# hungdinhxuan/real-time-deepfake-speech-detection

Hardware: AMD Instinct MI355X
Metric: utterances/sec (4 s @ 16 kHz) (higher is better)
Workload: dtype fp16

## Files before the change

### real-time-deepfake-speech-detection_amd/csrc/afx_engine.hip

```cpp
#include <hip/hip_runtime.h>

#include <algorithm>
#include <cmath>
#include <cstdarg>
#include <cstdio>
#include <cstring>
#include <string>
#include <unordered_map>
#include <unordered_set>
#include <vector>

#include "../../include/afx.h"
#include "afx_common.h"
#include "afx_kernels.h"
#include "afx_aasist.h"
#include "afx_entry.h"

using namespace afx;

static thread_local char g_err[512] = "";
int afx::fail(const char* fmt, ...) {
  va_list ap;
  va_start(ap, fmt);
  vsnprintf(g_err, sizeof g_err, fmt, ap);
// ... 29 lines not shown
  for (int i = 0; i < 7; ++i) {
    L = L >= kConvK[i] ? (L - kConvK[i]) / kConvS[i] + 1 : 0;
    T[i] = L;
  }
}

__global__ void bn_fold_kernel(const float* w, const float* b, const float* m, const float* v, float eps, int n,
                               float* scale, float* shift) {
  const int i = blockIdx.x * blockDim.x + threadIdx.x;
  if (i < n) {
    const float s = w[i] / sqrtf(v[i] + eps);
    scale[i] = s;
    shift[i] = b[i] - m[i] * s;
  }
}

__global__ void absmax_kernel(const float* x, int n, float* out) {
  float m = 0.f;
  for (int i = threadIdx.x; i < n; i += blockDim.x) m = fmaxf(m, fabsf(x[i]));
  __shared__ float red[4];
  m = wave_max(m);
  if ((threadIdx.x & 63) == 0) red[threadIdx.x >> 6] = m;
  __syncthreads();
  if (threadIdx.x == 0) out[0] = fmaxf(fmaxf(red[0], red[1]), fmaxf(red[2], red[3]));
}

struct FT {
  float* p = nullptr;
  size_t n = 0;
  std::vector<int64_t> shape;
};

struct TapRec {
  float* p = nullptr;
  size_t cap = 0, n = 0;
};

struct LnW {
  const float *g = nullptr, *b = nullptr;
  float scale = kS3ScaleBounded;
};
struct ConvLayer {
  const float* bias = nullptr;
  LnW ln;
  const float *w0 = nullptr, *gn_g = nullptr, *gn_b = nullptr;
};
struct TrunkLayer {
  void *wqkv = nullptr, *wo = nullptr, *w1 = nullptr, *w2 = nullptr;
  float* bqkv = nullptr;
  LnW ln1, ln2;
  const float *bo = nullptr, *b1 = nullptr, *b2 = nullptr;
};
struct ConfFF {
  void *w1, *w2;
  LnW ln;
  const float *b1, *b2;
};
struct ConfBlock {
  ConfFF ff[2];
  void *wqkv, *wout, *pw1, *pw2;
  float *bn_scale, *bn_shift;
  void* rel_h;
  float* chain_prm[3];
  LnW attn_ln, conv_ln, post_ln;
  const float *bout, *bpw1, *bpw2;
  const float* rel32;
  const float *dw_w, *dw_b;
};

struct Profiler;

struct afx_engine {
  afx_config cfg;
  bool s3 = false;
  Profiler* prof = nullptr;
  int dt;
  size_t hsz;
  std::vector<void*> allocs;
  std::unordered_map<std::string, FT> f;
  std::unordered_set<std::string> loaded;
  bool finalized = false;
  bool taps_on = false;
  int posconv_sliding = 1;
  int conf_attn_mfma = 1;
  int fuse_conformer = 1;
  int fuse_conv_ln = 1;
  int gemm_small_deep = 1;
  int concurrent = 0;
  int last_objective = 0;
  std::unordered_map<std::string, TapRec> taps;
  int* nonfinite = nullptr;

  void* convw[7] = {nullptr};
  void* conv0pack = nullptr;
  void* projw = nullptr;
  void* posw = nullptr;
  float* pos_norm = nullptr;
  ConvLayer conv[7];
  LnW feat_ln, enc_ln;
  const float *proj_b = nullptr, *pos_b = nullptr;
  std::vector<TrunkLayer> layers;
  int E = 0, Ep = 0, heads = 0, dh = 0, inner = 0, FF = 0, FFp = 0, C2 = 0, C2p = 0, ck = 0, nblk = 0;
  void* conf_ll = nullptr;
  float conf_bn_scale = 1.f, conf_bn_shift = 0.f;
  const float *ll_b = nullptr, *class_token = nullptr, *fc5_w = nullptr, *fc5_b = nullptr;
  std::vector<ConfBlock> blk;
  AasistWeights aw;

  void* walloc(size_t rows, size_t k) { return dalloc(rows * k * hsz + (s3 ? rows * 4 : 0)); }
  float* wscale(const void* w, size_t rows, size_t k) const { return s3 ? (float*)((char*)w + rows * k * 4) : nullptr; }
  void* dalloc(size_t bytes) {
    void* p = nullptr;
    if (hipMalloc(&p, bytes ? bytes : 16) != hipSuccess) return nullptr;
    allocs.push_back(p);
    return p;
  }
  const float* F(const std::string& k) const {
    auto it = f.find(k);
    return it == f.end() ? nullptr : it->second.p;
  }
};

static void prof_forget(afx_engine* e);
extern "C" const char* afx_last_error(void) { return g_err; }
extern "C" const char afx_build_id_str[];
extern "C" const char* afx_build_id(void) { return afx_build_id_str; }
extern "C" const char* afx_version(void) {
  static char v[96] = "";
  if (!v[0]) snprintf(v, sizeof v, "afx 0.4 (gfx950) build %s hip %d.%d.%d", afx_build_id_str, HIP_VERSION_MAJOR, HIP_VERSION_MINOR, HIP_VERSION_PATCH);
  return v;
}
extern "C" int afx_hip_versions(int* build, int* runtime) {
  if (build) *build = HIP_VERSION;
  int rt = 0;
  if (hipRuntimeGetVersion(&rt) != hipSuccess) return fail("afx_hip_versions: hipRuntimeGetVersion failed");
  if (runtime) *runtime = rt;
  return 0;
}

extern "C" int afx_create(const afx_config* cfg, afx_handle* out) {
  if (!cfg || !out) return fail("afx_create: null argument");
  const bool head_only = cfg->arch == AFX_ARCH_CONFORMER_HEAD;
  if (!head_only && (cfg->n_layers < 1 || cfg->n_layers > 24))
    return fail("Number of layers must be at least 1 and at most 24.");
  if (cfg->dtype != AFX_DT_BF16 && cfg->dtype != AFX_DT_FP16 && cfg->dtype != AFX_DT_FP32 && cfg->dtype != AFX_DT_FP16X3)
    return fail("afx_create: unknown dtype %d", cfg->dtype);
  if (cfg->arch < AFX_ARCH_SSL || cfg->arch > AFX_ARCH_CONFORMER_HEAD) return fail("afx_create: unknown arch %d", cfg->arch);
  if (cfg->extractor_mode != AFX_EXTRACTOR_LAYER_NORM && cfg->extractor_mode != AFX_EXTRACTOR_GROUP_NORM)
    return fail("afx_create: unknown extractor_mode %d", cfg->extractor_mode);
  if (cfg->extractor_mode == AFX_EXTRACTOR_GROUP_NORM && cfg->pre_emphasis)
    return fail("afx_create: fused pre-emphasis is built for the layer_norm extractor only");
  int ndev = 0;
  if (hipGetDeviceCount(&ndev) != hipSuccess || ndev == 0)
    return fail("afx_create: no HIP device visible -- this library has no CPU fallback");
  afx_engine* e = new afx_engine();
  e->cfg = *cfg;
  e->s3 = cfg->dtype == AFX_DT_FP16X3;
  e->dt = e->s3 ? (int)DT_FP32 : cfg->dtype;
  e->hsz = dtype_size(e->dt);
  const int nl = head_only ? 0 : cfg->n_layers;
  e->cfg.n_layers = nl;
  e->layers.resize(nl);
  bool ok = true;
  ok &= (e->nonfinite = (int*)e->dalloc(16)) != nullptr && hipMemset(e->nonfinite, 0, 16) == hipSuccess;
  if (!head_only) {
    for (int i = 1; i < 7; ++i) ok &= (e->convw[i] = e->walloc(kC, (size_t)kC * kConvK[i])) != nullptr;
// ... 820 lines not shown
  const hipStream_t s = cx.s;
  const int dt = e->dt;
  const int* T = w.T;
  if (T[6] < 1) return fail("afx_forward: %d samples are too few for one output frame (need >= 400)", L);
  const ConvLayer& c0 = e->conv[0];
  const bool gn = e->cfg.extractor_mode == AFX_EXTRACTOR_GROUP_NORM;
  if (!l5)
    KOK(cx.timed(PC_CONV0, 2.0 * B * T[0] * kC * kConvK[0], [&] {
      if (gn)
        return launch_conv0_groupnorm(wave, B, L, T[0], c0.w0, c0.gn_g, c0.gn_b, kLnEps,
                                      w.gn_stats, w.bufA, dt, s);
      if (e->s3) {
        const float sc = cx.s3_ok(w.bufA) ? c0.ln.scale : 0.f;
        cx.s3_set(w.bufA, sc);
        return launch_conv0(wave, B, L, T[0], c0.w0, c0.bias, c0.ln.g, c0.ln.b, e->cfg.pre_emphasis, e->cfg.pre_emphasis_coef, w.bufA, DT_FP16X3, s, e->conv0pack, sc);
      }
      return launch_conv0(wave, B, L, T[0], c0.w0, c0.bias, c0.ln.g, c0.ln.b, e->cfg.pre_emphasis, e->cfg.pre_emphasis_coef, w.bufA, dt, s,
                          e->conv0pack);
    }));
  if (!l5) TAP("c0", w.bufA, (size_t)B * T[0] * kC, true, kC);
  void* in = l5 ? const_cast<void*>(l5) : w.bufA;
  void* out = w.bufB;
  for (int i = l5 ? 6 : 1; i < 7; ++i) {
    const int M = B * T[i], K = kConvK[i] * kC;
    GemmArgs g = plain_gemm(in, 0, e->convw[i], K, M, kC, K);
    g.rpb = T[i]; g.a_batch = (l5 && i == 6 && l5_batch) ? l5_batch : (long)T[i - 1] * kC; g.a_row = (long)kConvS[i] * kC;
    g.o_batch_rows = T[i]; g.oh_batch_rows = T[i];
    g.bias = e->conv[i].bias;
    g.act = ACT_GELU;
    if (gn) {
      if (i < 6) {
        g.out_h = out; g.ldo_h = kC;
      } else {
        g.out_f = w.tmp32; g.ldo_f = kC;
      }
      KOK(cx.gemm(g, dt, 1));
    } else if (e->fuse_conv_ln && dt != DT_FP32) {
      g.ln_gamma = e->conv[i].ln.g; g.ln_beta = e->conv[i].ln.b; g.ln_eps = kLnEps;
      if (i < 6) {
        g.out_h = out; g.ldo_h = kC;
      } else {
        g.out_f = w.tmp32; g.ldo_f = kC;
      }
      KOK(cx.gemm(g, dt, 1));
    } else {
      g.act = ACT_NONE;
      g.out_f = w.tmp32; g.ldo_f = kC;
      KOK(cx.gemm(g, dt, 1));
      RowNormArgs n = plain_norm(w.tmp32, kC, M, kC);
      n.act = ACT_GELU;
      if (i < 6) {
        n.out_h = out; n.ldo_h = kC;
      } else {
        n.out_f = w.tmp32; n.ldo_f = kC;
      }
      KOK(cx.rownorm(n, e->conv[i].ln, dt));
    }
    if (i < 6) TAP("c" + std::to_string(i), out, (size_t)M * kC, true, kC);
    void* t = in; in = out; out = t;
  }
  const int Tt = T[6], M = B * Tt;
  if (tap(cx, "conv", w.tmp32, (size_t)M * kC, false)) return 1;
  {
    RowNormArgs n = plain_norm(w.tmp32, kC, M, kC);
    n.out_h = w.feats_h; n.ldo_h = kC;
    KOK(cx.rownorm(n, e->feat_ln, dt));
  }
  TAP("feats", w.feats_h, (size_t)M * kC, true, kC);
  {
    GemmArgs g = plain_gemm(w.feats_h, kC, e->projw, kC, M, kD, kC);
    g.rpb = Tt; g.a_batch = (long)Tt * kC; g.a_row = kC;
    g.bias = e->proj_b;
    g.out_f = w.x; g.ldo_f = kD; g.o_batch_rows = Tt; g.o_row_off = 0;
    g.out_h = w.xpad; g.ldo_h = kD; g.oh_batch_rows = Tt + kPosK; g.oh_row_off = kPosPad;
    KOK(cx.gemm(g, dt, 1));
    KOK(cx.timed(PC_MISC, 0, [&] { return launch_zero_pad_rows(w.xpad, B, Tt, kD, kPosPad, kPosK - kPosPad, dt, s, w.lens); }));
  }
  TAP("xpad", w.xpad, (size_t)B * (Tt + kPosK) * kD, true, kD);
  if (tap(cx, "proj", w.x, (size_t)M * kD, false)) return 1;
  if (e->posconv_sliding && dt != DT_FP32 && Tt <= 224) {
    PosConvArgs pc;
    memset(&pc, 0, sizeof pc);
    pc.xpad = w.xpad; pc.xpad_batch = (long)(Tt + kPosK) * kD; pc.W = e->posw; pc.bias = e->pos_b;
    pc.x = w.x; pc.B = B; pc.T = Tt;
    KOK(cx.timed(PC_POSCONV, 2.0 * M * kD * (kD / kPosG) * kPosK, [&] { return launch_posconv(pc, dt, s); }));
  } else {
    KOK(posconv_product(cx, w.xpad, Tt + kPosK, B, Tt, w.x, dt));
  }
  if (tap(cx, "pos", w.x, (size_t)M * kD, false)) return 1;
  auto resid_product = [&](const void* A, long lda, const void* W, int K, const float* bias) -> const char* {
    GemmArgs o = plain_gemm(A, lda, W, K, M, kD, K);
    o.bias = bias; o.resid = w.x; o.ldr = kD; o.out_f = w.x; o.ldo_f = kD;
    return cx.gemm(o, dt, 1);
  };
  for (int l = 0; l < e->cfg.n_layers; ++l) {
    const TrunkLayer& L = e->layers[l];
    RowNormArgs n1 = plain_norm(w.x, kD, M, kD);
    n1.out_h = w.hbuf; n1.ldo_h = kD;
    KOK(cx.rownorm(n1, L.ln1, dt));
    auto lp = [l](const char* leaf) { return "l" + std::to_string(l) + "." + leaf; };
    TAP(lp("ln1"), w.hbuf, (size_t)M * kD, true, kD);
    GemmArgs q = plain_gemm(w.hbuf, kD, L.wqkv, kD, M, 3 * kD, kD);
    q.bias = L.bqkv;
    q.out_h = w.qkv; q.ldo_h = 3 * kD;
    KOK(cx.gemm(q, dt, 1));
    TAP(lp("qkv"), w.qkv, (size_t)M * 3 * kD, true, 3 * kD);
    KOK(cx.timed(PC_MHSA, 4.0 * B * kH * (double)Tt * Tt * 64, [&] {
      if (e->s3 && Tt <= 224) {
        const bool pairs = cx.s3_ok(w.att);
        cx.s3_set(w.att, pairs ? kS3ScaleFree : 0.f);
        return launch_mhsa_split((const float*)w.qkv, (float*)w.att, B, Tt, kH, s, w.lens, pairs, kS3ScaleFree);
      }
      if (e->s3) cx.s3_set(w.att, 0.f);
      return launch_mhsa(w.qkv, w.att, B, Tt, kH, dt, s, w.lens);
    }));
    TAP(lp("att"), w.att, (size_t)M * kD, true, kD);
    KOK(resid_product(w.att, kD, L.wo, kD, L.bo));
    TAP(lp("mid"), w.x, (size_t)M * kD, false, kD);
    RowNormArgs n2 = plain_norm(w.x, kD, M, kD);
    n2.out_h = w.hbuf; n2.ldo_h = kD;
    KOK(cx.rownorm(n2, L.ln2, dt));
    TAP(lp("ln2"), w.hbuf, (size_t)M * kD, true, kD);
    GemmArgs f1 = plain_gemm(w.hbuf, kD, L.w1, kD, M, kF, kD);
    f1.bias = L.b1; f1.act = ACT_GELU;
    f1.out_h = w.ff; f1.ldo_h = kF;
    KOK(cx.gemm(f1, dt, 1));
    TAP(lp("ff"), w.ff, (size_t)M * kF, true, kF);
    KOK(resid_product(w.ff, kF, L.w2, kF, L.b2));
    if (e->taps_on) {
      const std::string nm = "layer" + std::to_string(l);
      if (tap(cx, nm.c_str(), w.x, (size_t)M * kD, false)) return 1;
    }
  }
  RowNormArgs nf = plain_norm(w.x, kD, M, kD);
  nf.out_f = w.ssl_f; nf.ldo_f = kD;
  nf.out_h = w.ssl_h; nf.ldo_h = kD;
  nf.nonfinite = e->nonfinite;
  nf.nf_lens = w.lens; nf.nf_rpb = Tt;
  KOK(cx.rownorm(nf, e->enc_ln, dt));
  if (tap(cx, "ssl", w.ssl_f, (size_t)M * kD, false)) return 1;
  TAP("ssl.op", w.ssl_h, (size_t)M * kD, true, kD);
  return 0;
}

static int run_conformer(Call& cx, int B, int T, Ws& w, float* logits, const float* tokens = nullptr, float* embedding = nullptr) {
  afx_engine* e = cx.e;
  const hipStream_t s = cx.s;
  const int dt = e->dt, E = e->E, Ep = e->Ep, N = T + 1, M = B * N;
  if (tokens) {
    KOK(cx.timed(PC_MISC, 0, [&] { return launch_conf_tokens(tokens, e->class_token, 1.f, 0.f, B, T, E, w.xc, s, true); }));
  } else {
    GemmArgs ll = plain_gemm(w.ssl_h, kD, e->conf_ll, kD, B * T, E, kD);
    ll.bias = e->ll_b;
    ll.out_f = w.ll32; ll.ldo_f = E;
    KOK(cx.gemm(ll, dt, 1));
    KOK(cx.timed(PC_MISC, 0, [&] {
      return launch_conf_tokens(w.ll32, e->class_token, e->conf_bn_scale, e->conf_bn_shift, B, T, E, w.xc, s);
    }));
  }
  if (tap(cx, "tokens", w.xc, (size_t)M * E, false)) return 1;
  const size_t hs = dtype_size(dt);
  const bool fused = e->fuse_conformer && (dt != DT_FP32 || e->s3) && E == 144 && e->inner == E && e->FFp == 4 * E && e->C2 == 2 * E;
  const int chain_dt = e->s3 ? DT_FP16X3 : dt;
  HIP_OK(hipMemsetAsync(w.ao, 0, (size_t)M * Ep * hs, s));
  if (!fused) {
    HIP_OK(hipMemsetAsync(w.hc, 0, (size_t)M * Ep * hs, s));
    HIP_OK(hipMemsetAsync(w.u, 0, (size_t)M * e->C2p * hs, s));
// ... 308 lines not shown
}
__global__ void kv_scatter_logits_kernel(const float* __restrict__ in, const int* __restrict__ ids, int nb, float* __restrict__ logits) {
  const int i = blockIdx.x * blockDim.x + threadIdx.x;
  if (i < nb * 2) logits[(long)ids[i >> 1] * 2 + (i & 1)] = in[i];
}

static int kv_to_per_stream(afx_kv* k, hipStream_t s) {
  if (k->per_stream) return 0;
  std::vector<int> t((size_t)k->S * 8, 0);
  for (int b = 0; b < k->S; ++b)
    for (int g = 0; g < kKvGroups; ++g) ((unsigned char*)&t[(size_t)b * 8 + 4])[g] = (unsigned char)k->cnt[g];
  HIP_OK(hipMemcpyAsync(k->tab, t.data(), t.size() * 4, hipMemcpyHostToDevice, s));
  HIP_OK(hipStreamSynchronize(s));
  k->nfeat_s.assign(k->S, k->nfeat);
  k->hmeta.assign((size_t)k->S * 4, 0);
  k->per_stream = true;
  return 0;
}

extern "C" int afx_kv_reset(afx_kv* k, const int* slots, int n_slots, void* stream) {
  if (!k || (n_slots > 0 && !slots) || n_slots < 0) return fail("afx_kv_reset: bad argument");
  std::vector<char> seen(k->S, 0);
  for (int i = 0; i < n_slots; ++i) {
    if (slots[i] < 0 || slots[i] >= k->S) return fail("afx_kv_reset: slot %d outside 0..%d", slots[i], k->S - 1);
    if (seen[slots[i]]++) return fail("afx_kv_reset: slot %d named twice", slots[i]);
  }
  hipStream_t s = (hipStream_t)stream;
  if (kv_to_per_stream(k, s)) return 1;
  if (n_slots == 0) return 0;
  for (int i = 0; i < n_slots; ++i) {
    k->nfeat_s[slots[i]] = 0;
    k->hmeta[(size_t)3 * k->S + i] = slots[i];
  }
  int* dslots = k->meta + 3 * k->S;
  HIP_OK(hipMemcpyAsync(dslots, k->hmeta.data() + 3 * k->S, (size_t)n_slots * 4, hipMemcpyHostToDevice, s));
  HIP_OK(hipStreamSynchronize(s));
  const size_t hs = k->e->hsz;
  hipLaunchKernelGGL(kv_reset_kernel, dim3(64, n_slots), dim3(256), 0, s, dslots, k->tab, k->active ? -1 : (int)(k->hop % kKvGroups), (u32x4*)k->hist,
                     (long)(kKvHist * kD * hs / 16), (u32x4*)k->feat[0], (u32x4*)k->feat[1], (long)(kKvFeat * kD * 4 / 16));
  HIP_OK(hipGetLastError());
  return 0;
}

struct KvCalls {
  Call chunk, head;
  KvCalls(afx_engine* e, void* stream, const KvWs& w)
      : chunk(e, stream, w.s3planes, w.s3bytes, {w.feats_h, w.hbuf, w.att, w.ff, w.xpad, (char*)w.xpad + (size_t)kKvHist * kD * e->hsz}),
        head(e, stream, w.head) {}
};
static int kv_trunk(Call& cx, afx_kv* k, const KvForm& f, const float* feats6, int n, KvWs& w) {
  afx_engine* e = cx.e;
  const hipStream_t s = cx.s;
  const int R = f.rows, dt = e->dt, M = R * n, Tp = kKvHist + n;
  const size_t hs = e->hsz, xrow = (size_t)kD * hs, xpad_pitch = (size_t)(Tp + kPosK) * xrow;
  {
    RowNormArgs a = plain_norm(feats6, kC, M, kC);
    a.out_h = w.feats_h; a.ldo_h = kC;
    KOK(cx.rownorm(a, e->feat_ln, dt));
  }
  TAP("kv.feats", w.feats_h, (size_t)M * kC, true, kC);
  if (f.ids) {
    hipLaunchKernelGGL(kv_hist_kernel, dim3(32, R), dim3(256), 0, s, (u32x4*)k->hist, (u32x4*)w.xpad, f.dn, (long)(xrow / 16),
                       (long)(Tp + kPosK), kPosPad, f.ids, 1);
    HIP_OK(hipGetLastError());
  } else {
    HIP_OK(hipMemcpy2DAsync((char*)w.xpad + kPosPad * xrow, xpad_pitch, k->hist, kKvHist * xrow, kKvHist * xrow, R, hipMemcpyDeviceToDevice, s));
  }
  {
    GemmArgs g = plain_gemm(w.feats_h, kC, e->projw, kC, M, kD, kC);
    g.rpb = n; g.a_batch = (long)n * kC; g.a_row = kC;
    g.bias = e->proj_b;
    g.out_f = w.x; g.ldo_f = kD; g.o_batch_rows = n;
    g.out_h = w.xpad; g.ldo_h = kD; g.oh_batch_rows = Tp + kPosK; g.oh_row_off = kPosPad + kKvHist;
    KOK(cx.gemm(g, dt, 1));
    KOK(cx.timed(PC_MISC, 0, [&] { return launch_zero_pad_rows(w.xpad, R, Tp, kD, kPosPad, kPosK - kPosPad, dt, s, f.pad_lens); }));
  }
  TAP("kv.xpad", w.xpad, (size_t)R * (Tp + kPosK) * kD, true, kD);
  TAP("kv.proj", w.x, (size_t)M * kD, false, kD);
  void* xchunk = (char*)w.xpad + (size_t)kKvHist * xrow;
  if (!e->s3) {
    PosConvArgs pc;
    memset(&pc, 0, sizeof pc);
    pc.xpad = xchunk; pc.xpad_batch = (long)(Tp + kPosK) * kD; pc.W = e->posw; pc.bias = e->pos_b;
    pc.x = w.x; pc.B = R; pc.T = n;
    KOK(cx.timed(PC_POSCONV, 2.0 * R * n * kD * (kD / kPosG) * kPosK, [&] { return launch_posconv(pc, dt, s); }));
  } else {
    cx.s3_set(xchunk, kS3ScaleFree);
    KOK(posconv_product(cx, xchunk, Tp + kPosK, R, n, w.x, dt));
  }
  TAP("kv.pos", w.x, (size_t)M * kD, false, kD);
  if (f.dn) {
    hipLaunchKernelGGL(kv_hist_kernel, dim3(32, R), dim3(256), 0, s, (u32x4*)k->hist, (u32x4*)w.xpad, f.dn, (long)(xrow / 16),
                       (long)(Tp + kPosK), kPosPad, f.ids, 0);
    HIP_OK(hipGetLastError());
  } else {
    HIP_OK(hipMemcpy2DAsync(k->hist, kKvHist * xrow, (char*)w.xpad + (size_t)(kPosPad + n) * xrow, xpad_pitch, kKvHist * xrow, R, hipMemcpyDeviceToDevice, s));
  }
  for (int l = 0; l < e->cfg.n_layers; ++l) {
    const TrunkLayer& L = e->layers[l];
    void* ring = (char*)k->rings + (size_t)l * k->S * kKvSlots * 3 * kD * hs;
    auto lp = [l](const char* leaf) { return "kv.l" + std::to_string(l) + "." + leaf; };
    RowNormArgs n1 = plain_norm(w.x, kD, M, kD);
    n1.out_h = w.hbuf; n1.ldo_h = kD;
    KOK(cx.rownorm(n1, L.ln1, dt));
    TAP(lp("ln1"), w.hbuf, (size_t)M * kD, true, kD);
    GemmArgs q = plain_gemm(w.hbuf, kD, L.wqkv, kD, M, 3 * kD, kD);
    q.rpb = n; q.a_batch = (long)n * kD; q.a_row = kD;
    q.bias = L.bqkv;
    q.out_h = ring; q.ldo_h = 3 * kD;
    if (f.qkv_rows) {
      q.oh_rows = f.qkv_rows;
    } else {
      q.oh_batch_rows = kKvSlots; q.oh_row_off = f.ring.q_tile * 16;
    }
    KOK(cx.gemm(q, dt, 1, f.qkv_rows != nullptr));
    TAP(lp("ring"), ring, (size_t)k->S * kKvSlots * 3 * kD, true, 3 * kD);
    KOK(cx.timed(PC_MHSA, 4.0 * R * kH * 16.0 * kKvSlots * 64, [&] {
      if (e->s3) {
        const bool pairs = cx.s3_ok(w.att);
        cx.s3_set(w.att, pairs ? kS3ScaleFree : 0.f);
        return launch_mhsa_ring_split((const float*)ring, (float*)w.att, R, kH, f.ring, s, pairs, kS3ScaleFree);
      }
      return launch_mhsa_ring(ring, w.att, R, kH, f.ring, dt, s);
    }));
    TAP(lp("att"), w.att, (size_t)R * 16 * kD, true, kD);
    GemmArgs o = plain_gemm(w.att, kD, L.wo, kD, M, kD, kD);
    o.rpb = n; o.a_batch = 16L * kD; o.a_row = kD; o.o_batch_rows = n;
    o.bias = L.bo; o.resid = w.x; o.ldr = kD; o.out_f = w.x; o.ldo_f = kD;
    KOK(cx.gemm(o, dt, 1));
    TAP(lp("mid"), w.x, (size_t)M * kD, false, kD);
    RowNormArgs n2 = plain_norm(w.x, kD, M, kD);
    n2.out_h = w.hbuf; n2.ldo_h = kD;
    KOK(cx.rownorm(n2, L.ln2, dt));
    TAP(lp("ln2"), w.hbuf, (size_t)M * kD, true, kD);
    GemmArgs f1 = plain_gemm(w.hbuf, kD, L.w1, kD, M, kF, kD);
    f1.bias = L.b1; f1.act = ACT_GELU; f1.out_h = w.ff; f1.ldo_h = kF;
    KOK(cx.gemm(f1, dt, 1));
    TAP(lp("ff"), w.ff, (size_t)M * kF, true, kF);
    GemmArgs f2 = plain_gemm(w.ff, kF, L.w2, kF, M, kD, kF);
    f2.bias = L.b2; f2.resid = w.x; f2.ldr = kD; f2.out_f = w.x; f2.ldo_f = kD;
    KOK(cx.gemm(f2, dt, 1));
    TAP("kv.layer" + std::to_string(l), w.x, (size_t)M * kD, false, kD);
  }
  RowNormArgs nf = plain_norm(w.x, kD, M, kD);
  if (f.win_next) {
    const size_t frow = (size_t)kD * 4, fpitch = (size_t)kKvFeat * frow;
    HIP_OK(hipMemcpy2DAsync(f.win_next, fpitch, (char*)k->feat[k->pp] + (size_t)n * frow, fpitch, (size_t)(kKvFeat - n) * frow, R, hipMemcpyDeviceToDevice, s));
    nf.out_f = f.win_next; nf.ldo_f = kD; nf.rpb = n; nf.o_batch_rows = kKvFeat; nf.o_row_off = kKvFeat - n;
  } else {
    nf.out_f = w.fl; nf.ldo_f = kD;
  }
  nf.nonfinite = e->nonfinite;
  KOK(cx.rownorm(nf, e->enc_ln, dt));
  if (!f.win_next) TAP("kv.fl", w.fl, (size_t)M * kD, false, kD);
  return 0;
}

extern "C" int afx_kv_step(afx_kv* k, const float* feats6, int n, float* logits, void* ws, size_t ws_bytes, void* stream) {
  if (n < 1 || n > 16) return fail("afx_kv_step: a chunk brings 1..16 frames (got %d)", n);
  if (!k || !feats6 || !logits || !ws) return fail("afx_kv_step: null argument");
  if (k->active) return fail("afx_kv_step: this state holds per-stream ring positions (afx_kv_step_active): continue with afx_kv_step_active");
  if (k->per_stream) return fail("afx_kv_step: this state holds per-stream sessions (afx_kv_reset / afx_kv_step_ragged): continue with afx_kv_step_ragged");
  afx_engine* e = k->e;
  const int S = k->S, dt = e->dt, group = (int)(k->hop % kKvGroups);
  const int Th = std::min(k->nfeat + n, kKvWindow);
  if (e->cfg.arch == AFX_ARCH_XLSR_AASIST && Th < 6) return fail("afx_kv_step: the AASIST head needs at least 6 frames in the window");
  KvWs w;
// ... 758 lines not shown
  }
  if (!strcmp(key, "gemm_s3_small")) {
    gemm_set_s3_small(value);
    return 0;
  }
  if (!strcmp(key, "gemm_split")) {
    gemm_set_split(value);
    return 0;
  }
  if (!strcmp(key, "gemm_conv_split")) {
    gemm_set_conv_split(value);
    return 0;
  }
  if (!strcmp(key, "gemm_ph4")) {
    gemm_set_ph4(value);
    return 0;
  }
  if (!strcmp(key, "gemm_fit")) {
    gemm_set_fit(value);
    return 0;
  }
  if (!strcmp(key, "dispatch_objective")) {
    dispatch_force_objective(value);
    return 0;
  }
  if (!strcmp(key, "dispatch_cu_mask")) {
    dispatch_set_cu_mask(value);
    return 0;
  }
  if (!strcmp(key, "conf_chain_waves")) {
    conf_chain_set_waves(value);
    return 0;
  }
  if (!strcmp(key, "conf_attn_waves")) {
    conf_attn_mfma_set_waves(value);
    return 0;
  }
  if (!strcmp(key, "mhsa_vtr")) {
    mhsa_set_vtr(value);
    return 0;
  }
  if (!strcmp(key, "mhsa_zsplit")) {
    mhsa_set_zsplit(value);
    return 0;
  }
  if (!strcmp(key, "mhsa_waves")) {
    mhsa_set_waves(value);
    return 0;
  }
  if (!strcmp(key, "mhsa_force_long")) {
    mhsa_set_force_long(value);
    return 0;
  }
  if (!strcmp(key, "conf_attn_force_long")) {
    conf_attn_mfma_set_force_long(value);
    return 0;
  }
  if (!strcmp(key, "conf_attn_block")) {
    conf_attn_set_block(value);
    return 0;
  }
  if (!strcmp(key, "gemm_deep")) {
    gemm_set_deep(value);
    return 0;
  }
  if (!strcmp(key, "gemm_nodma")) {
    if (!gemm_set_nodma(value)) return fail("afx_debug_set: gemm_nodma exists only in the attribution build (make attr, AFX_LIB=.../libafx_attr.so)");
    return 0;
  }
  if (!strcmp(key, "gemm_a_nt")) {
    gemm_set_a_nt(value);
    return 0;
  }
  if (!strcmp(key, "conv0_mfma")) {
    conv0_set_mfma(value);
    return 0;
  }

  return fail("afx_debug_set: unknown key '%s'", key);
}
extern "C" int afx_engine_set(afx_handle h, const char* key, int value) {
  if (!h || !key) return fail("afx_engine_set: null argument");
  if (!strcmp(key, "posconv_sliding")) h->posconv_sliding = value != 0;
  else if (!strcmp(key, "conf_attn_mfma")) h->conf_attn_mfma = value != 0;
  else if (!strcmp(key, "fuse_conformer")) h->fuse_conformer = value != 0;
  else if (!strcmp(key, "fuse_conv_ln")) h->fuse_conv_ln = value != 0;
  else if (!strcmp(key, "gemm_small_deep")) h->gemm_small_deep = value != 0;
  else if (!strcmp(key, "concurrent")) h->concurrent = value != 0;
  else return fail("afx_engine_set: unknown key '%s'", key);
  return 0;
}
extern "C" int afx_engine_get(afx_handle h, const char* key, int* value) {
  if (!h || !key || !value) return fail("afx_engine_get: null argument");
  if (!strcmp(key, "concurrent")) *value = h->concurrent;
  else if (!strcmp(key, "objective")) *value = h->last_objective;
  else return fail("afx_engine_get: unknown key '%s'", key);
  return 0;
}
extern "C" int afx_gemm_plan(int M, int N, int K, int rpb, int kchunk, int groups, int flags, int objective, int* out) {
  if (!out || M <= 0 || N <= 0 || K <= 0 || groups <= 0) return fail("afx_gemm_plan: bad arguments");
  GemmArgs g = plain_gemm(nullptr, K, nullptr, K, M, N, K);
  if (rpb > 0) g.rpb = rpb;
  if (kchunk > 0) g.kchunk = kchunk;
  if (flags & 1) g.ln_gamma = g.ln_beta = g.bias = (const float*)out;
  if (flags & 2) { g.k1 = K; g.K = 2 * K; g.kchunk = 2 * g.kchunk; }
  if (flags & 4) g.act = ACT_SWISH;
  if (flags & 8) g.no_deep = 1;
  const int obj = objective < 0 ? dispatch_objective(OBJ_MAKESPAN) : (objective ? OBJ_CU_TIME : OBJ_MAKESPAN);
  const GemmPlan pl = gemm_plan(g, groups, obj);
  out[0] = pl.family; out[1] = pl.tile; out[2] = pl.rows; out[3] = (int)pl.tiles;
  out[4] = pl.split_rows; out[5] = pl.rem_tile; out[6] = (int)pl.rem_tiles; out[7] = obj;
  return 0;
}
extern "C" int afx_conf_chain_waves(int M, int objective) {
  return conf_chain_waves_of(M, objective < 0 ? dispatch_objective(OBJ_MAKESPAN) : (objective ? OBJ_CU_TIME : OBJ_MAKESPAN));
}
extern "C" int afx_k_pre_emphasis(const float* x, int B, int L, float coef, float* y, void* stream) {
  KRET(launch_pre_emphasis(x, B, L, coef, y, (hipStream_t)stream));
}
extern "C" int afx_k_tile_crop(const float* x, const long long* offs, const long long* starts, int B, int duration,
                               float* out, void* stream) {
  if (!x || !offs || !out) return fail("afx_k_tile_crop: null argument");
  KRET(launch_tile_crop(x, offs, starts, B, duration, out, (hipStream_t)stream));
}
extern "C" int afx_k_rownorm(int dtype, const float* x, long ldx, int rows, int C, const float* gamma,
                             const float* beta, float eps, int act, float* out_f, long ldo_f, void* out_h, long ldo_h,
                             void* stream) {
  RowNormArgs a = plain_norm(x, ldx, rows, C);
  a.gamma = gamma; a.beta = beta; a.eps = eps; a.act = act; a.out_f = out_f; a.ldo_f = ldo_f; a.out_h = out_h; a.ldo_h = ldo_h;
  KRET(launch_rownorm(a, dtype, (hipStream_t)stream));
}
extern "C" int afx_k_mhsa(int dtype, const void* qkv, void* out, int B, int T, int H, void* stream) {
  if (dtype == DT_FP16X3) KRET(launch_mhsa_split((const float*)qkv, (float*)out, B, T, H, (hipStream_t)stream));
  KRET(launch_mhsa(qkv, out, B, T, H, dtype, (hipStream_t)stream));
}
extern "C" int afx_k_conf_attn(int dtype, const float* q, long ldq, const float* kv, long ldkv, const float* rel,
                               int max_pos, int B, int N, int H, int dh, void* out_h, long ldo, void* stream) {
  KRET(launch_conf_attn(q, ldq, kv, ldkv, rel, max_pos, B, N, H, dh, out_h, ldo, dtype, (hipStream_t)stream));
}
extern "C" int afx_k_conf_attn_mfma(int dtype, const float* q, long ldq, const float* kv, long ldkv, const void* rel_h,
                                    int max_pos, int B, int N, int H, int dh, void* out_h, long ldo, void* stream) {
  if (dtype == DT_FP16X3)
    KRET(launch_conf_attn_split(q, ldq, kv, ldkv, (const float*)rel_h, max_pos, B, N, H, dh, (float*)out_h, ldo, (hipStream_t)stream));
  KRET(launch_conf_attn_mfma(q, ldq, kv, ldkv, rel_h, max_pos, B, N, H, dh, out_h, ldo, dtype, (hipStream_t)stream));
}
extern "C" int afx_k_conf_dwconv(int dtype, const float* x, long ldx, const float* w, const float* bias,
                                 const float* bn_scale, const float* bn_shift, int B, int N, int C, int k, void* out_h,
                                 long ldo, void* stream) {
  KRET(launch_conf_dwconv(x, ldx, w, bias, bn_scale, bn_shift, B, N, C, k, out_h, ldo, dtype, (hipStream_t)stream));
}
```

### real-time-deepfake-speech-detection_amd/csrc/afx_kernels.h

```cpp
#pragma once
#include <hip/hip_runtime.h>
#include <stdint.h>

namespace afx {

enum DType { DT_BF16 = 0, DT_FP16 = 1, DT_FP32 = 2, DT_FP16X3 = 3 };
inline size_t dtype_size(int dt) { return dt == DT_FP32 || dt == DT_FP16X3 ? 4 : 2; }
constexpr float kS3ScaleBounded = 16.f;
constexpr float kS3ScaleFree = 1.f;
__host__ __device__ inline long s3_pair_index(long k) { return ((k >> 5) << 6) + (k & 31); }

struct GemmArgs {
  const void* A;
  const void* W;
  int M, N, K;
  int k_algo;
  int rpb;
  long a_batch, a_row;
  int kchunk;
  long kchunk_stride;
  long ldw;
  long g_a, g_w;
  int g_n;
  const float* bias;
// ... 34 lines not shown
int gemm_tile_of(const GemmArgs& p, int groups);
enum { OBJ_MAKESPAN = 0, OBJ_CU_TIME = 1 };
enum { CU_GEMM8_HEIGHT = 1, CU_CHAIN_WAVES = 2, CU_ROWLN_HEIGHT = 4, CU_SPLITS = 8 };
void dispatch_force_objective(int obj);
void dispatch_set_cu_mask(int mask);
int dispatch_objective(int of_launch);
bool dispatch_cu(int obj, int bit);
struct GemmPlan {
  int family;
  int tile;
  int rows;
  long tiles;
  int split_rows;
  int rem_tile;
  long rem_tiles;
};
GemmPlan gemm_plan(const GemmArgs& p, int groups, int objective);
void gemm_set_s3_small(int v);
void gemm_set_map_mode(int m);
void gemm_set_small_deep(int v);
void gemm_set_tile(int t);
void gemm_set_a_nt(int v);
void gemm_set_conv_split(int v);
void gemm_set_ph4(int v);
void gemm_set_fit(int v);
void gemm_set_split(int v);
void mhsa_set_zsplit(int v);
void mhsa_set_waves(int v);
void mhsa_set_force_long(int v);
void conf_attn_mfma_set_waves(int v);
void conf_attn_mfma_set_force_long(int v);
void conf_attn_set_block(int v);
void gemm_set_deep(int v);
bool gemm_set_nodma(int v);

const char* launch_conv0(const float* wave, int B, int L, int T0, const float* w ,
                         const float* bias, const float* gamma, const float* beta, int pre_emph,
                         float pre_coef, void* out_h, int dtype, hipStream_t s, const void* wpack = nullptr, float pair_scale = 0.f);
size_t conv0_pack_bytes();
const char* launch_conv0_pack(const float* w , const float* bias, void* pack, hipStream_t s);
const char* launch_conv0_groupnorm(const float* wave, int B, int L, int T0, const float* w, const float* gamma,
                                   const float* beta, float eps, float* stats, void* out_h, int dtype, hipStream_t s);
size_t conv0_groupnorm_stats_floats(int B, int T0);
const char* launch_tile_crop(const float* x, const long long* offs, const long long* starts, int B, int duration,
                             float* out, hipStream_t s);
void conv0_set_mfma(int v);
const char* launch_pre_emphasis(const float* x, int B, int L, float coef, float* y, hipStream_t s);
struct RowNormArgs {
  const float* x;
  long ldx;
  int rows, C;
  const float* gamma;
  const float* beta;
  float eps;
  int act;
  float* out_f;
  long ldo_f;
  void* out_h;
  long ldo_h;
  int rpb, o_batch_rows, o_row_off;
  int* nonfinite;
  const int* nf_lens;
  int nf_rpb;
  int oh_pairs;
  float oh_scale;
};
const char* launch_rownorm(const RowNormArgs& a, int dtype, hipStream_t s);
const char* launch_zero_pad_rows(void* buf_h, int B, int T, int C, int pad_front, int pad_back, int dtype,
                                 hipStream_t s, const int* lens = nullptr);
const char* launch_pack_linear(const float* w, int N, int K, int Kpad, void* out_h, int dtype, hipStream_t s);
const char* launch_pack_conv(const float* w, int N, int Cin, int k, void* out_h, int dtype, hipStream_t s);
const char* launch_pack_posconv(const float* v, const float* g, int C, int cpg, int k, float* norm_tmp ,
                                void* out_h, int dtype, hipStream_t s);
const char* launch_split_weight_rows(void* w_f32_inplace, int N, int K, float* row_scale, hipStream_t s);
const char* launch_split_pairs(const float* x, long n, void* pairs, float scale, hipStream_t s);

struct PosConvArgs {
  const void* xpad;
  long xpad_batch;
  const void* W;
  const float* bias;
  float* x;
  int B, T, slab_rows;
};
const char* launch_posconv(const PosConvArgs& p, int dtype, hipStream_t s);

const char* launch_mhsa(const void* qkv, void* out, int B, int T, int H, int dtype, hipStream_t s, const int* lens = nullptr);
void mhsa_set_vtr(int v);

const char* launch_mhsa_split(const float* qkv, float* out, int B, int T, int H, hipStream_t s, const int* lens = nullptr,
                              bool out_pairs = false, float out_scale = 1.f);
struct MhsaRingForm {
  int form;
  int q_tile;
  const int* cnt;
  const int* tab;
};
const char* launch_mhsa_ring(const void* ring, void* out, int S, int H, const MhsaRingForm& f, int dtype, hipStream_t s);
const char* launch_mhsa_ring_split(const float* ring, float* out, int S, int H, const MhsaRingForm& f, hipStream_t s,
                                   bool out_pairs = false, float out_scale = 1.f);

const char* launch_conf_tokens(const float* ll, const float* cls, float bn_scale, float bn_shift, int B, int T,
                               int E, float* out, hipStream_t s, bool raw = false);
const char* launch_conf_attn(const float* q, long ldq, const float* kv, long ldkv, const float* rel, int max_pos,
                             int B, int N, int H, int dh, void* out_h, long ldo, int dtype, hipStream_t s,
                             const int* lens = nullptr, int len_add = 0);
const char* launch_conf_attn_split(const float* q, long ldq, const float* kv, long ldkv, const float* rel64, int max_pos, int B, int N,
                                   int H, int dh, float* out, long ldo, hipStream_t s, const int* lens = nullptr, int len_add = 0);
const char* launch_conf_attn_mfma(const float* q, long ldq, const float* kv, long ldkv, const void* rel_h, int max_pos,
                                  int B, int N, int H, int dh, void* out_h, long ldo, int dtype, hipStream_t s,
                                  const int* lens = nullptr, int len_add = 0);
const char* launch_conf_dwconv(const float* x, long ldx, const float* w , const float* bias,
                               const float* bn_scale, const float* bn_shift, int B, int N, int C, int k,
                               void* out_h, long ldo, int dtype, hipStream_t s, const int* lens = nullptr, int len_add = 0);
enum ChainParamOffsets { CP_FF_G = 0, CP_FF_B = 144, CP_FF_B1 = 288, CP_FF_B2 = 864, CP_LN2_G = 1008, CP_LN2_B = 1152,
                         CP_BA = 1296, CP_BB = 1440 };
constexpr int kChainParamFloats = 2048;
constexpr int kChainScaleFloats = 2048;
enum ChainScaleOffsets { CS_FF1 = 0, CS_FF2 = 576, CS_A = 720, CS_B = 1152 };
static_assert(CS_B + 576 <= kChainScaleFloats, "scale block");
struct ConfChainArgs {
  int M, E, Ep, FFp;
  const float* x_in;
  float* x_out;
  const float* params;
  const void *ff_w1, *ff_w2;
  const void* w_a;
  int ld_w_a;
  int objective;
  const void* w_b;
  const void* in_h;
  long ld_in_h;
  float* out2;
  long ld_out2;
};
const char* launch_conf_chain(const ConfChainArgs& p, int stage, int dtype, hipStream_t s);
void conf_chain_set_waves(int v);
int conf_chain_waves_of(int M, int objective);
const char* launch_small_linear(const float* x, long row_stride, int rows, int K, const float* w, const float* b,
                                int N, float* out, hipStream_t s, int* nonfinite = nullptr);

}
```

### real-time-deepfake-speech-detection_amd/csrc/afx_posconv.hip

```cpp
#include "afx_common.h"
#include "afx_kernels.h"

namespace afx {

namespace {
constexpr int PC_C = 1024, PC_CPG = 64, PC_TAPS = 128, PC_RING = 4, PC_NW = 8, PC_MAXT = 4;
}

template <class HT>
__global__ __launch_bounds__(64 * PC_NW) void posconv_kernel(PosConvArgs p) {
  typedef typename HT::T T;
  typedef typename HT::V8 V8;
  extern __shared__ __attribute__((aligned(16))) char smem[];
  const int tid = threadIdx.x, lane = tid & 63;
  const int wave = __builtin_amdgcn_readfirstlane(tid >> 6);
  const int l15 = lane & 15, kq = lane >> 4;
  const int rows = p.slab_rows;
  const int slab_bytes = rows * 128;
  char* ring = smem + 2 * slab_bytes;
  const unsigned lds_base = (unsigned)(size_t)smem;
  const int id = blockIdx.x, k2 = id >> 3;
  const int grp = (id & 7) * 2 + (k2 & 1), pair = k2 >> 1;
  const int u0 = pair * 2;
  const int nslot = u0 + 1 < p.B ? 2 : 1;
  const T* xp = (const T*)p.xpad;
  const T* wg = (const T*)p.W + (long)grp * PC_CPG * (PC_CPG * PC_TAPS);

  auto dma16 = [&](const T* src, unsigned off) {
    unsigned keep;
    const unsigned dst = __builtin_amdgcn_readfirstlane(lds_base + off);
    asm volatile("s_mov_b32 %0, m0\n\ts_mov_b32 m0, %2\n\ts_nop 0\n\tglobal_load_lds_dwordx4 %1, off\n\ts_mov_b32 m0, %0"
                 : "=&s"(keep) : "v"(src), "s"(dst) : "memory");
  };
  const int last_row = p.T + PC_TAPS - 1;
  for (int s = 0; s < nslot; ++s) {
    const T* xb = xp + (long)(u0 + s) * p.xpad_batch + grp * PC_CPG;
    for (int q = wave; q < rows / 8; q += PC_NW) {
      int row = q * 8 + (lane >> 3);
      const int c = (lane & 7) ^ (((row >> 1) & 3) << 1);
      row = row < last_row ? row : last_row;
      dma16(xb + (long)row * PC_C + c * 8, s * slab_bytes + q * 1024);
    }
  }
  auto issue_tap = [&](int j) {
    static_assert(PC_NW == 8, "one 8-row piece of the 64-row weight tile per wave");
    const int row = wave * 8 + (lane >> 3);
    const int c = (lane & 7) ^ ((row >> 1) & 7);
    dma16(wg + (long)row * (PC_CPG * PC_TAPS) + j * PC_CPG + c * 8, 2 * slab_bytes + (j & (PC_RING - 1)) * 8192 + wave * 1024);
  };
  issue_tap(0);
  issue_tap(1);
  issue_tap(2);

  const int nrt = (p.T + 15) >> 4, ntiles = nslot * nrt;
  int abase[PC_MAXT], aoff[PC_MAXT];
#pragma unroll
  for (int i = 0; i < PC_MAXT; ++i) {
    const int q = wave + PC_NW * i;
    const int slot = q >= nrt ? 1 : 0, rt = q - slot * nrt;
    abase[i] = rt * 16 + l15;
    aoff[i] = slot * slab_bytes;
  }
  f32x4 acc[PC_MAXT][4];
#pragma unroll
  for (int i = 0; i < PC_MAXT; ++i)
#pragma unroll
    for (int c = 0; c < 4; ++c) acc[i][c] = f32x4{0.f, 0.f, 0.f, 0.f};
  const int wsw = (l15 >> 1) & 7;
  const int woff[2] = {l15 * 128 + ((kq ^ wsw) * 16), l15 * 128 + (((4 + kq) ^ wsw) * 16)};

  for (int j = 0; j < PC_TAPS; ++j) {
    if (j + 2 < PC_TAPS) asm volatile("s_waitcnt vmcnt(2)" ::: "memory");
    else if (j + 1 < PC_TAPS) asm volatile("s_waitcnt vmcnt(1)" ::: "memory");
    else asm volatile("s_waitcnt vmcnt(0)" ::: "memory");
    __builtin_amdgcn_s_barrier();
    asm volatile("" ::: "memory");
    if (j + 3 < PC_TAPS) issue_tap(j + 3);
    const char* wb = ring + (j & (PC_RING - 1)) * 8192;
    V8 wf[4][2];
#pragma unroll
    for (int c = 0; c < 4; ++c)
#pragma unroll
      for (int ks = 0; ks < 2; ++ks) wf[c][ks] = *(const V8*)(wb + c * 2048 + woff[ks]);
#pragma unroll
    for (int i = 0; i < PC_MAXT; ++i) {
      if (wave + PC_NW * i < ntiles) {
        const int R = abase[i] + j;
        const int sw = ((R >> 1) & 3) << 1;
        const V8 a0 = *(const V8*)(smem + aoff[i] + R * 128 + ((kq ^ sw) * 16));
        const V8 a1 = *(const V8*)(smem + aoff[i] + R * 128 + (((4 + kq) ^ sw) * 16));
#pragma unroll
        for (int c = 0; c < 4; ++c) acc[i][c] = HT::mfma(wf[c][0], a0, acc[i][c]);
#pragma unroll
        for (int c = 0; c < 4; ++c) acc[i][c] = HT::mfma(wf[c][1], a1, acc[i][c]);
      }
    }
  }

#pragma unroll
  for (int i = 0; i < PC_MAXT; ++i) {
    const int q = wave + PC_NW * i;
    if (q >= ntiles) continue;
    const int slot = q >= nrt ? 1 : 0, rt = q - slot * nrt;
    const int t = rt * 16 + l15;
    if (t >= p.T) continue;
    float* xr = p.x + ((long)(u0 + slot) * p.T + t) * PC_C + grp * PC_CPG;
    f32x4 bv[4], rv[4];
#pragma unroll
    for (int c = 0; c < 4; ++c) {
      const int col = c * 16 + kq * 4;
      bv[c] = *(const f32x4*)(p.bias + grp * PC_CPG + col);
      rv[c] = *(const f32x4*)(xr + col);
    }
#pragma unroll
    for (int c = 0; c < 4; ++c) {
      const int col = c * 16 + kq * 4;
      *(f32x4*)(xr + col) = rv[c] + gelu_poly4(acc[i][c] + bv[c]);
    }
  }
}

const char* launch_posconv(const PosConvArgs& p_in, int dtype, hipStream_t s) {
  PosConvArgs p = p_in;
  if (dtype == DT_FP32) return "posconv: half-precision operands only (exact mode uses the fp32 GEMM)";
  if (p.B <= 0 || p.T <= 0 || 2 * ((p.T + 15) / 16) > PC_NW * PC_MAXT || p.T > 224) return "posconv: 1..224 frames";
  p.slab_rows = (p.T + PC_TAPS - 1 + 7) & ~7;
  const int lds = 2 * p.slab_rows * 128 + PC_RING * 8192;
  if (lds > 160 * 1024) return "posconv: slab does not fit the LDS";
  static LdsLimit lim[2];
  hipError_t e = hipSuccess;
  const int npair = (p.B + 1) / 2;
  dim3 grid(16 * npair);
  if (dtype == DT_BF16) {
    e = lim[0].ensure((const void*)posconv_kernel<BF16>, lds);
    if (e == hipSuccess) hipLaunchKernelGGL(posconv_kernel<BF16>, grid, dim3(64 * PC_NW), lds, s, p);
  } else {
    e = lim[1].ensure((const void*)posconv_kernel<FP16>, lds);
    if (e == hipSuccess) hipLaunchKernelGGL(posconv_kernel<FP16>, grid, dim3(64 * PC_NW), lds, s, p);
  }
  if (e == hipSuccess) e = hipGetLastError();
  return e == hipSuccess ? nullptr : hipGetErrorString(e);
}

}
```

Measured before the change: 13780.

## Software-pipeline posconv LDS fragment reads with MFMA and deepen tap prefetch

Adds a pipelined variant of the grouped positional convolution kernel, enabled by default. It double-buffers the weight and activation fragments in registers, so LDS reads for tap j+1 are interleaved with the MFMAs of tap j under sched barriers. It also prefetches four taps ahead instead of three and specialises the loop on the number of tiles each wave owns. The goal is to hide LDS latency behind matrix math, at the cost of more register pressure and more template instantiations. Only the posconv stage is affected, which is a small part of the whole model.

```diff
diff --git a/real-time-deepfake-speech-detection_amd/csrc/afx_engine.hip b/real-time-deepfake-speech-detection_amd/csrc/afx_engine.hip
--- a/real-time-deepfake-speech-detection_amd/csrc/afx_engine.hip
+++ b/real-time-deepfake-speech-detection_amd/csrc/afx_engine.hip
@@ -135,6 +135,7 @@
   bool finalized = false;
   bool taps_on = false;
   int posconv_sliding = 1;
+  int posconv_pipe = 1;
   int conf_attn_mfma = 1;
   int fuse_conformer = 1;
   int fuse_conv_ln = 1;
@@ -1121,7 +1122,7 @@
     PosConvArgs pc;
     memset(&pc, 0, sizeof pc);
     pc.xpad = w.xpad; pc.xpad_batch = (long)(Tt + kPosK) * kD; pc.W = e->posw; pc.bias = e->pos_b;
-    pc.x = w.x; pc.B = B; pc.T = Tt;
+    pc.x = w.x; pc.B = B; pc.T = Tt; pc.pipe = e->posconv_pipe;
     KOK(cx.timed(PC_POSCONV, 2.0 * M * kD * (kD / kPosG) * kPosK, [&] { return launch_posconv(pc, dt, s); }));
   } else {
     KOK(posconv_product(cx, w.xpad, Tt + kPosK, B, Tt, w.x, dt));
@@ -1596,7 +1597,7 @@
     PosConvArgs pc;
     memset(&pc, 0, sizeof pc);
     pc.xpad = xchunk; pc.xpad_batch = (long)(Tp + kPosK) * kD; pc.W = e->posw; pc.bias = e->pos_b;
-    pc.x = w.x; pc.B = R; pc.T = n;
+    pc.x = w.x; pc.B = R; pc.T = n; pc.pipe = e->posconv_pipe;
     KOK(cx.timed(PC_POSCONV, 2.0 * R * n * kD * (kD / kPosG) * kPosK, [&] { return launch_posconv(pc, dt, s); }));
   } else {
     cx.s3_set(xchunk, kS3ScaleFree);
@@ -2521,6 +2522,7 @@
 extern "C" int afx_engine_set(afx_handle h, const char* key, int value) {
   if (!h || !key) return fail("afx_engine_set: null argument");
   if (!strcmp(key, "posconv_sliding")) h->posconv_sliding = value != 0;
+  else if (!strcmp(key, "posconv_pipe")) h->posconv_pipe = value != 0;
   else if (!strcmp(key, "conf_attn_mfma")) h->conf_attn_mfma = value != 0;
   else if (!strcmp(key, "fuse_conformer")) h->fuse_conformer = value != 0;
   else if (!strcmp(key, "fuse_conv_ln")) h->fuse_conv_ln = value != 0;
diff --git a/real-time-deepfake-speech-detection_amd/csrc/afx_kernels.h b/real-time-deepfake-speech-detection_amd/csrc/afx_kernels.h
--- a/real-time-deepfake-speech-detection_amd/csrc/afx_kernels.h
+++ b/real-time-deepfake-speech-detection_amd/csrc/afx_kernels.h
@@ -140,6 +140,7 @@
   const float* bias;
   float* x;
   int B, T, slab_rows;
+  int pipe;
 };
 const char* launch_posconv(const PosConvArgs& p, int dtype, hipStream_t s);
 
diff --git a/real-time-deepfake-speech-detection_amd/csrc/afx_posconv.hip b/real-time-deepfake-speech-detection_amd/csrc/afx_posconv.hip
--- a/real-time-deepfake-speech-detection_amd/csrc/afx_posconv.hip
+++ b/real-time-deepfake-speech-detection_amd/csrc/afx_posconv.hip
@@ -1,13 +1,17 @@
 #include "afx_common.h"
 #include "afx_kernels.h"
+#include <type_traits>
 
 namespace afx {
 
 namespace {
 constexpr int PC_C = 1024, PC_CPG = 64, PC_TAPS = 128, PC_RING = 4, PC_NW = 8, PC_MAXT = 4;
-}
-
-template <class HT>
+constexpr int PC_WAIT_LDS = 0xC07F;
+template <int V>
+using pc_int = std::integral_constant<int, V>;
+}
+
+template <class HT, bool PIPE>
 __global__ __launch_bounds__(64 * PC_NW) void posconv_kernel(PosConvArgs p) {
   typedef typename HT::T T;
   typedef typename HT::V8 V8;
@@ -51,6 +55,7 @@
   issue_tap(0);
   issue_tap(1);
   issue_tap(2);
+  if constexpr (PIPE) issue_tap(3);
 
   const int nrt = (p.T + 15) >> 4, ntiles = nslot * nrt;
   int abase[PC_MAXT], aoff[PC_MAXT];
@@ -69,32 +74,97 @@
   const int wsw = (l15 >> 1) & 7;
   const int woff[2] = {l15 * 128 + ((kq ^ wsw) * 16), l15 * 128 + (((4 + kq) ^ wsw) * 16)};
 
-  for (int j = 0; j < PC_TAPS; ++j) {
-    if (j + 2 < PC_TAPS) asm volatile("s_waitcnt vmcnt(2)" ::: "memory");
-    else if (j + 1 < PC_TAPS) asm volatile("s_waitcnt vmcnt(1)" ::: "memory");
-    else asm volatile("s_waitcnt vmcnt(0)" ::: "memory");
-    __builtin_amdgcn_s_barrier();
-    asm volatile("" ::: "memory");
-    if (j + 3 < PC_TAPS) issue_tap(j + 3);
-    const char* wb = ring + (j & (PC_RING - 1)) * 8192;
-    V8 wf[4][2];
-#pragma unroll
-    for (int c = 0; c < 4; ++c)
-#pragma unroll
-      for (int ks = 0; ks < 2; ++ks) wf[c][ks] = *(const V8*)(wb + c * 2048 + woff[ks]);
-#pragma unroll
-    for (int i = 0; i < PC_MAXT; ++i) {
-      if (wave + PC_NW * i < ntiles) {
-        const int R = abase[i] + j;
-        const int sw = ((R >> 1) & 3) << 1;
-        const V8 a0 = *(const V8*)(smem + aoff[i] + R * 128 + ((kq ^ sw) * 16));
-        const V8 a1 = *(const V8*)(smem + aoff[i] + R * 128 + (((4 + kq) ^ sw) * 16));
-#pragma unroll
-        for (int c = 0; c < 4; ++c) acc[i][c] = HT::mfma(wf[c][0], a0, acc[i][c]);
-#pragma unroll
-        for (int c = 0; c < 4; ++c) acc[i][c] = HT::mfma(wf[c][1], a1, acc[i][c]);
+  if constexpr (!PIPE) {
+    for (int j = 0; j < PC_TAPS; ++j) {
+      if (j + 2 < PC_TAPS) asm volatile("s_waitcnt vmcnt(2)" ::: "memory");
+      else if (j + 1 < PC_TAPS) asm volatile("s_waitcnt vmcnt(1)" ::: "memory");
+      else asm volatile("s_waitcnt vmcnt(0)" ::: "memory");
+      __builtin_amdgcn_s_barrier();
+      asm volatile("" ::: "memory");
+      if (j + 3 < PC_TAPS) issue_tap(j + 3);
+      const char* wb = ring + (j & (PC_RING - 1)) * 8192;
+      V8 wf[4][2];
+#pragma unroll
+      for (int c = 0; c < 4; ++c)
+#pragma unroll
+        for (int ks = 0; ks < 2; ++ks) wf[c][ks] = *(const V8*)(wb + c * 2048 + woff[ks]);
+#pragma unroll
+      for (int i = 0; i < PC_MAXT; ++i) {
+        if (wave + PC_NW * i < ntiles) {
+          const int R = abase[i] + j;
+          const int sw = ((R >> 1) & 3) << 1;
+          const V8 a0 = *(const V8*)(smem + aoff[i] + R * 128 + ((kq ^ sw) * 16));
+          const V8 a1 = *(const V8*)(smem + aoff[i] + R * 128 + (((4 + kq) ^ sw) * 16));
+#pragma unroll
+          for (int c = 0; c < 4; ++c) acc[i][c] = HT::mfma(wf[c][0], a0, acc[i][c]);
+#pragma unroll
+          for (int c = 0; c < 4; ++c) acc[i][c] = HT::mfma(wf[c][1], a1, acc[i][c]);
+        }
       }
     }
+  } else {
+    static_assert(PC_MAXT == 4 && PC_RING == 4, "tile slot i carries the reads of weight tile c = i; tap j+4 refills the slot of tap j");
+    auto taps = [&](auto NT_) {
+      constexpr int NT = decltype(NT_)::value;
+      V8 wf[2][4][2], af[2][PC_MAXT][2];
+      auto read_slot = [&](int j, int i, auto S_) {
+        constexpr int S = decltype(S_)::value;
+        if constexpr (NT > 0) {
+          const char* wb = ring + (j & (PC_RING - 1)) * 8192 + i * 2048;
+          wf[S][i][0] = *(const V8*)(wb + woff[0]);
+          wf[S][i][1] = *(const V8*)(wb + woff[1]);
+        }
+        if (i < NT) {
+          const int R = abase[i] + j;
+          const int sw = ((R >> 1) & 3) << 1;
+          af[S][i][0] = *(const V8*)(smem + aoff[i] + R * 128 + ((kq ^ sw) * 16));
+          af[S][i][1] = *(const V8*)(smem + aoff[i] + R * 128 + (((4 + kq) ^ sw) * 16));
+        }
+      };
+      auto step = [&](int j, auto S_, auto VM_, auto DMA_) {
+        constexpr int S = decltype(S_)::value, VM = decltype(VM_)::value;
+        __builtin_amdgcn_s_waitcnt(PC_WAIT_LDS);
+        if constexpr (VM >= 0) {
+          if constexpr (VM == 2) asm volatile("s_waitcnt vmcnt(2)" ::: "memory");
+          else if constexpr (VM == 1) asm volatile("s_waitcnt vmcnt(1)" ::: "memory");
+          else asm volatile("s_waitcnt vmcnt(0)" ::: "memory");
+          __builtin_amdgcn_s_barrier();
+          asm volatile("" ::: "memory");
+          if constexpr (decltype(DMA_)::value) issue_tap(j + 4);
+        }
+#pragma unroll
+        for (int i = 0; i < PC_MAXT; ++i) {
+          if constexpr (VM >= 0) read_slot(j + 1, i, pc_int<1 - S>{});
+          __builtin_amdgcn_sched_barrier(0);
+          if (i < NT) {
+#pragma unroll
+            for (int c = 0; c < 4; ++c) acc[i][c] = HT::mfma(wf[S][c][0], af[S][i][0], acc[i][c]);
+#pragma unroll
+            for (int c = 0; c < 4; ++c) acc[i][c] = HT::mfma(wf[S][c][1], af[S][i][1], acc[i][c]);
+          }
+          __builtin_amdgcn_sched_barrier(0);
+        }
+      };
+      asm volatile("s_waitcnt vmcnt(3)" ::: "memory");
+      __builtin_amdgcn_s_barrier();
+      asm volatile("" ::: "memory");
+#pragma unroll
+      for (int i = 0; i < PC_MAXT; ++i) read_slot(0, i, pc_int<0>{});
+      for (int j = 0; j < PC_TAPS - 4; j += 2) {
+        step(j, pc_int<0>{}, pc_int<2>{}, pc_int<1>{});
+        step(j + 1, pc_int<1>{}, pc_int<2>{}, pc_int<1>{});
+      }
+      step(PC_TAPS - 4, pc_int<0>{}, pc_int<2>{}, pc_int<0>{});
+      step(PC_TAPS - 3, pc_int<1>{}, pc_int<1>{}, pc_int<0>{});
+      step(PC_TAPS - 2, pc_int<0>{}, pc_int<0>{}, pc_int<0>{});
+      step(PC_TAPS - 1, pc_int<1>{}, pc_int<-1>{}, pc_int<0>{});
+    };
+    const int own = (ntiles - wave + PC_NW - 1) >> 3;
+    if (own >= 4) taps(pc_int<4>{});
+    else if (own == 3) taps(pc_int<3>{});
+    else if (own == 2) taps(pc_int<2>{});
+    else if (own == 1) taps(pc_int<1>{});
+    else taps(pc_int<0>{});
   }
 
 #pragma unroll
@@ -127,16 +197,20 @@
   p.slab_rows = (p.T + PC_TAPS - 1 + 7) & ~7;
   const int lds = 2 * p.slab_rows * 128 + PC_RING * 8192;
   if (lds > 160 * 1024) return "posconv: slab does not fit the LDS";
-  static LdsLimit lim[2];
+  static LdsLimit lim[4];
   hipError_t e = hipSuccess;
   const int npair = (p.B + 1) / 2;
   dim3 grid(16 * npair);
+  auto go = [&](auto kernel, LdsLimit& l) {
+    e = l.ensure((const void*)kernel, lds);
+    if (e == hipSuccess) hipLaunchKernelGGL(kernel, grid, dim3(64 * PC_NW), lds, s, p);
+  };
   if (dtype == DT_BF16) {
-    e = lim[0].ensure((const void*)posconv_kernel<BF16>, lds);
-    if (e == hipSuccess) hipLaunchKernelGGL(posconv_kernel<BF16>, grid, dim3(64 * PC_NW), lds, s, p);
+    if (p.pipe) go(posconv_kernel<BF16, true>, lim[0]);
+    else go(posconv_kernel<BF16, false>, lim[1]);
   } else {
-    e = lim[1].ensure((const void*)posconv_kernel<FP16>, lds);
-    if (e == hipSuccess) hipLaunchKernelGGL(posconv_kernel<FP16>, grid, dim3(64 * PC_NW), lds, s, p);
+    if (p.pipe) go(posconv_kernel<FP16, true>, lim[2]);
+    else go(posconv_kernel<FP16, false>, lim[3]);
   }
   if (e == hipSuccess) e = hipGetLastError();
   return e == hipSuccess ? nullptr : hipGetErrorString(e);
```

New measurement: 13770 (median of 3 runs). Within noise of the previous version (-0.0%).
